# FedeMont/collision_handling_in_instantNGP

Measured on AMD Instinct MI355X. Metric: Mpixels/sec fwd+bwd at L=16,F=2,T=2^19, higher is better.
Workload: dtype f32

## Files before the change

collision_handling_in_instantngp_amd/_lib.py:

```python
import ctypes
import os

import torch

_HERE = os.path.dirname(os.path.abspath(__file__))
LIB_PATH = os.environ.get("GNGF_LIB_PATH") or os.path.join(_HERE, "libgngf_hip.so")

_c = ctypes
_P = _c.c_void_p
_I = _c.c_int
_L = _c.c_int64
_F = _c.c_float
_D = _c.c_double

SIGNATURES = {
    "gngf_abi_version": [],
    "gngf_hash_indices": [_P, _P, _P, _L, _I, _L, _P],
    "gngf_mrhe_fwd": [_P, _I, _P, _P, _P, _L, _I, _I, _L, _I, _I, _P],
    "gngf_mrhe_bwd": [_P, _I, _P, _P, _P, _P, _P, _L, _I, _I, _L, _I, _I, _P],
    "gngf_bilinear_fwd": [_P, _P, _P, _P, _L, _I, _I, _P],
    "gngf_bilinear_bwd": [_P, _P, _P, _P, _L, _I, _I, _P],
    "gngf_encode_fwd": [_P, _P, _I, _P, _P, _P, _P, _L, _I, _I, _L, _I, _I, _I, _L, _I, _I, _P, _P],
    "gngf_encode_bwd": [_P, _P, _I, _P, _P, _P, _P, _P, _P, _L, _I, _I, _L, _I, _I, _I, _L, _I, _I, _P],
    "gngf_encode_bwd_bucketed_plan": [_L, _I, _L, _I, _I, _P],
    "gngf_encode_bwd_bucketed": [_P, _P, _P, _P, _L, _I, _I, _L, _I, _I, _I, _I, _P, _P, _P, _P, _P],
    "gngf_clear_hashed_rows": [_P, _P, _I, _I, _L, _L, _P],
    "gngf_bin_pixels": [_P, _L, _I, _I, _I, _P, _P, _P, _P, _P, _P, _P],
    "gngf_encode_tiled_prepare": [_P, _L, _I, _I, _I, _P, _P, _P, _P, _P, _P, _P, _I, _P, _P, _P, _P, _P, _P, _I, _I, _I, _L, _I, _I, _I, _L,
                                  _P, _L, _P, _P, _P],
    "gngf_vertex_grid_fwd": [_P, _I, _P, _P, _P, _P, _P, _I, _I, _L, _I, _I, _I, _L, _P],
    "gngf_vertex_grid_bwd": [_P, _I, _P, _P, _P, _P, _P, _P, _P, _I, _I, _L, _I, _I, _I, _L, _P],
    "gngf_encode_tiled_fwd": [_P, _P, _P, _I, _P, _P, _P, _P, _I, _I, _I, _I, _I, _P],
    "gngf_bin_pixels2": [_P, _P, _L, _P],
    "gngf_encode_tiled_fwd_fused": [_P, _P, _P, _I, _P, _P, _P, _I, _P, _P, _P, _I, _I, _I, _L, _I, _I, _I, _L, _I, _I, _P, _P],
    "gngf_set_tiled_interleaved": [_I],
    "gngf_tiled_interleaved_applies": [_P, _I, _I, _I, _I, _I],
    "gngf_debug_il_stamps": [_P],
    "gngf_encode_tiled_bwd": [_P, _P, _P, _I, _P, _P, _P, _P, _P, _P, _I, _I, _P, _P, _I, _I, _I, _I, _I, _I,
                              _P, _P, _P, _P, _P, _P, _P, _L, _I, _I, _P, _P, _P, _P, _P, _P, _L, _P, _L, _P, _I, _P, _P],
    "gngf_vertex_grid_bwd_sorted": [_P, _I, _P, _P, _P, _P, _P, _P, _L, _P, _P, _I, _I, _L, _I, _I, _L, _P],
    "gngf_decoder_fwd": [_P, _P, _P, _P, _P, _P, _P, _P, _P, _L, _I, _I, _I, _P],
    "gngf_decoder_bwd": [_P, _P, _P, _P, _P, _P, _P, _P, _P, _P, _P, _P, _P, _P, _P, _P, _P, _P, _P, _P, _P, _L, _L, _I, _I, _I, _P],
    "gngf_decoder_reduce": [_P, _P, _P, _P, _P, _P, _P, _P, _P, _P, _L, _I, _I, _P],
    "gngf_decoder_train": [_P] * 20 + [_L, _L, _I, _I, _I, _P],
    "gngf_decoder_bwd_last_span_ns": [_P],
    "gngf_decoder_hidden_floats": [_L],
    "gngf_decoder_bwd_slabs": [_L],
    "gngf_decoder_slab_floats": [_I, _I],
    "gngf_set_gemm_split_bf16": [_I],
    "gngf_set_decoder_bwd_hybrid": [_I],
    "gngf_linear_fwd": [_P, _P, _P, _P, _L, _I, _I, _I, _P],
    "gngf_linear_bwd_input": [_P, _P, _P, _P, _L, _I, _I, _I, _P],
    "gngf_linear_bwd_weight": [_P, _P, _P, _P, _P, _L, _I, _I, _I, _P],
    "gngf_gemm_acc": [_P, _P, _P, _L, _L, _L, _I, _I, _P],
    "gngf_softmax_topk": [_P, _P, _P, _P, _L, _L, _I, _P],
    "gngf_softmax_bwd_lowrank": [_P, _P, _P, _P, _P, _P, _I, _P, _P, _P, _L, _L, _I, _P],
    "gngf_hpd_bwd_dot": [_P, _P, _P, _P, _P, _P, _I, _P, _L, _L, _I, _P],
    "gngf_hpd_bwd_fused_applies": [_L, _L, _I, _I, _I],
    "gngf_hpd_bwd_prepare": [_P, _P, _L, _P, _P, _P, _P, _L, _P, _P, _I, _I, _I, _P],
    "gngf_hpd_bwd_fused": [_P] * 8 + [_L, _P, _P, _P, _P, _P, _P, _P, _L, _L, _I, _I, _I, _P],
    "gngf_logits_topk_pbar": [_P, _P, _P, _P, _P, _I, _P, _L, _L, _I, _P],
    "gngf_linear_fwd_rowstats": [_P, _P, _P, _P, _P, _L, _I, _I, _P],
    "gngf_rowstats_topk": [_P, _P, _P, _P, _P, _L, _L, _I, _P],
    "gngf_pbar_accumulate": [_P, _P, _P, _I, _P, _L, _L, _P],
    "gngf_topk": [_P, _P, _P, _L, _L, _I, _P],
    "gngf_softmax_bwd": [_P, _P, _P, _P, _P, _P, _I, _P, _L, _L, _I, _P],
    "gngf_vertex_coords": [_P, _L, _L, _I, _P],
    "gngf_blend_fwd": [_P, _P, _L, _I, _I, _P],
    "gngf_blend_bwd": [_P, _P, _P, _L, _I, _I, _P],
    "gngf_vertex_multiplicity": [_P, _P, _P, _L, _I, _I, _L, _P],
    "gngf_multiplicity_weights": [_P, _P, _L, _I, _F, _P],
    "gngf_expand_vertex_table": [_P, _P, _P, _P, _P, _P, _P, _L, _I, _I, _I, _L, _P],
    "gngf_mse_workspace_floats": [],
# ... 101 lines not shown
```

collision_handling_in_instantngp_amd/csrc/encode_tiled.hip:

```cpp
#include "gngf_common.h"

namespace gngf {

#ifndef GNGF_TBF
#define GNGF_TBF 512
#endif
#ifndef GNGF_TBB
#define GNGF_TBB 1024
#endif
constexpr int kTBF = GNGF_TBF;
constexpr int kTB = GNGF_TBB;
#ifndef GNGF_BIN_THREADS
#define GNGF_BIN_THREADS 1024
#endif
constexpr int kBinThreads = GNGF_BIN_THREADS;
constexpr int kBinU = 8;

__device__ __forceinline__ int g_max0(int v) { return v < 0 ? 0 : v; }

__device__ __forceinline__ int tile_of(float x, float y, int tile_shift) {
  const int TS = 1 << tile_shift;
  int tx = (int)(x * (float)TS), ty = (int)(y * (float)TS);
  tx = tx < 0 ? 0 : (tx >= TS ? TS - 1 : tx);
  ty = ty < 0 ? 0 : (ty >= TS ? TS - 1 : ty);
// ... 1501 lines not shown
      y = dppf<0x114, 0xF>(x); asm volatile("" : "+v"(y)); x += p4 ? y : 0.f;
      y = dppf<0x118, 0xF>(x); asm volatile("" : "+v"(y)); x += p8 ? y : 0.f;
      y = dppf<0x142, 0xA>(x); asm volatile("" : "+v"(y)); x += pA ? y : 0.f;
      y = dppf<0x143, 0xC>(x); asm volatile("" : "+v"(y)); x += pB ? y : 0.f;
      v[f] = x;
    }
    float (*tail)[F] = s_tail[l & 1];
    if (lane == 63) {
#pragma unroll
      for (int f = 0; f < F; ++f) tail[wave][f] = v[f];
    }
    __syncthreads();
    float carry[F];
#pragma unroll
    for (int f = 0; f < F; ++f) carry[f] = 0.f;
    for (int q = wave - 1; q >= 0; --q) {
      if (s_last[q] != first_key) break;
#pragma unroll
      for (int f = 0; f < F; ++f) carry[f] += tail[q][f];
      if (s_nruns[q] != 1) break;
    }
    if (emit) {
      float* d = dtables + ((int64_t)l * T + slot) * F;
#pragma unroll
      for (int f = 0; f < F; ++f) {
        const float tot = v[f] + (in_first_run ? carry[f] : 0.f);
        if (tot != 0.f) atomicAdd(d + f, tot);
      }
    }
  }
  if (live && dvert_w) dvert_w[e] = dw_acc;
}

}

using namespace gngf;

#define DISPATCH_TT(dt, ...)                                                          \
  if ((dt) == GNGF_FEAT_F32) { using TT = float; __VA_ARGS__; }                       \
  else if ((dt) == GNGF_FEAT_F16) { using TT = __half; __VA_ARGS__; }                 \
  else return (int)hipErrorInvalidValue;

#define DISPATCH_F(F, ...)                          \
  switch (F) {                                      \
    case 1: { constexpr int kF = 1; __VA_ARGS__; } break; \
    case 2: { constexpr int kF = 2; __VA_ARGS__; } break; \
    case 4: { constexpr int kF = 4; __VA_ARGS__; } break; \
    case 8: { constexpr int kF = 8; __VA_ARGS__; } break; \
    default: return (int)hipErrorInvalidValue;      \
  }

static bool bin_job_dev(const gngf_bin_job* j, bool reserving, BinJobDev* d) {
  if (!j || j->P < 0 || j->P >= (1ll << 31) || j->tile_shift < 0 || j->tile_shift > 6 || j->NB <= 0 || j->NB > kBinMaxBlocks || j->chunk <= 0)
    return false;
  if (!(j->xy && j->blockhist && j->tile_off && j->tile_item_base && j->items && j->n_items && j->sorted)) return false;
  if (reserving && !(j->P > 0 && j->persistent_ws)) return false;
  d->xy = reinterpret_cast<const float2*>(j->xy); d->P = j->P;
  d->per_block = ceil_div(ceil_div(j->P, j->NB), kBinThreads) * kBinThreads;
  d->NB = j->NB; d->tile_shift = j->tile_shift; d->chunk = j->chunk;
  d->blockhist = j->blockhist; d->pws = j->persistent_ws; d->tile_off = j->tile_off; d->tile_item_base = j->tile_item_base;
  d->items = reinterpret_cast<int4*>(j->items); d->n_items = j->n_items; d->sorted = reinterpret_cast<float4*>(j->sorted);
  return true;
}
static BinJobDev bin_job_none() {
  BinJobDev d = {nullptr, 0, 0, 0, 0, 0, nullptr, nullptr, nullptr, nullptr, nullptr, nullptr, nullptr};
  return d;
// ... 365 lines not shown
    if (max_items > 0 && !hdt_g) {
      if (hash_dtables)
        gather_partials_kernel<kF, true><<<dim3((unsigned)ceil_div(vtot_h, 256)), dim3(256), 0, as_stream(stream)>>>(
            partials, tile_item_base, tile_level_off, n_ls, dG, Ls, tile_shift, lds_bytes / 4, hash_dtables, hash_T, hpow2);
      else
        gather_partials_kernel<kF><<<dim3((unsigned)ceil_div(vtot_h, 256)), dim3(256), 0,
                                     as_stream(stream)>>>(partials, tile_item_base, tile_level_off, n_ls, dG, Ls, tile_shift,
                                                          lds_bytes / 4);
    }
  });
  GNGF_RETURN_LAUNCH();
}

extern "C" int gngf_vertex_grid_bwd_sorted(const void* tables, int feat_dtype, const int32_t* vert_idx, const float* vert_w,
                                           const int32_t* order, const int32_t* n_ls, const float* dG, const void* dG64,
                                           int64_t vtot, float* dtables, float* dvert_w, int Ls, int F, int64_t T, int K,
                                           int vstride, int64_t NV, void* stream) {
  GNGF_CHECK_ARG(Ls > 0 && Ls <= GNGF_MAX_LEVELS && T > 0 && K > 0 && K <= GNGF_MAX_TOPK && vstride > 0 && NV > 0);
  GNGF_CHECK_ARG(tables && vert_idx && vert_w && order && n_ls && (dG || (dG64 && vtot > 0)) && dtables && NV * K < (1ll << 31));
  const int64_t NE = NV * K;
  if (dG64) {
    DISPATCH_TT(feat_dtype, DISPATCH_F(F, (vertex_bwd_sorted_kernel<kF, TT, true><<<dim3((unsigned)ceil_div(NE, kVB)), dim3(kVB), 0,
                                                                                  as_stream(stream)>>>(
                                static_cast<const TT*>(tables), vert_idx, vert_w, order, n_ls, nullptr, dtables, dvert_w, Ls, T, K,
                                vstride, NE, static_cast<const unsigned long long*>(dG64), vtot))));
    GNGF_RETURN_LAUNCH();
  }
  DISPATCH_TT(feat_dtype, DISPATCH_F(F, (vertex_bwd_sorted_kernel<kF, TT, false><<<dim3((unsigned)ceil_div(NE, kVB)), dim3(kVB), 0,
                                                                                 as_stream(stream)>>>(
                              static_cast<const TT*>(tables), vert_idx, vert_w, order, n_ls, dG, dtables, dvert_w, Ls, T, K,
                              vstride, NE, nullptr, 0))));
  GNGF_RETURN_LAUNCH();
}
```

collision_handling_in_instantngp_amd/models.py:

```python
from typing import Tuple

import numpy as np
import torch
import torch.nn as nn

from . import ops
from .params import *

device = torch.device("cuda") if torch.cuda.is_available() else torch.device("cpu")

DENSE_OUTPUT_LIMIT_BYTES = 4 << 30
HPD_CHUNK_BYTES = 8 << 30


def level_resolutions(n_min: int, n_max: int, num_levels: int) -> np.ndarray:
    b = np.exp((np.log(n_max) - np.log(n_min)) / (num_levels - 1))
    return np.array([np.floor(n_min * b ** l) for l in range(num_levels)]).astype(np.int32)


class DifferentiableTopk(torch.autograd.Function):

    @staticmethod
    def forward(ctx, input: torch.Tensor, k: int, dim: int):
        if dim not in (-1, input.dim() - 1):
# ... 216 lines not shown
                self._fused_mse_target, self._fused_mse_gloss = prev
        return scope()

    def _vertex_extent(self, x):
        if self.coord_bounds is not None:
            mx, my = self.coord_bounds
        else:
            if x.shape[0] > 0:
                b = torch.cat([x.amax(0), -x.amin(0)])
            else:
                b = torch.zeros((4,), dtype=x.dtype, device=x.device)
            if self.dp.max_ is not None:
                self.dp.max_(b)
            mx, my, nx, ny = b.tolist()
            if nx > 0 or ny > 0:
                raise ValueError("GNGF indexing builds its per-vertex table over [0, max] x [0, max]: negative coordinates "
                                 f"(min {-nx:g}, {-ny:g}) are outside it")
        gx_hi = int(np.floor(np.float32(mx) * np.float32(self._n_max))) + 1
        gy_hi = int(np.floor(np.float32(my) * np.float32(self._n_max))) + 1
        return gx_hi + 1, (gx_hi + 1) * (gy_hi + 1)

    def hpd_is_frozen(self):
        return all(not p.requires_grad for p in self.HPD.parameters())

    @torch.no_grad()
    def _frozen_vertex_table(self, blend_code):
        params = self.HPD.flat_params()
        key = (tuple((p.data_ptr(), p._version) for p in params), blend_code, self._topk_k)
        if self._frozen_table is None or self._frozen_table[0] != key:
            vstride = self._n_max + 2
            NV = vstride * vstride
            tv, ti, _, _ = ops.HpdVertexFunction.apply(NV, vstride, self._topk_k, None, False, HPD_CHUNK_BYTES, None, *params)
            w = ops.BlendFunction.apply(tv, blend_code)
            self._frozen_table = (key, tv, ti, w, vstride, NV, ops.slot_order(ti, self._n_ls_host, vstride))
            if self._row_map is not None:
                self._mark_reachable_rows(ti, vstride, NV)
        return self._frozen_table[1:]

    @torch.no_grad()
    def _mark_reachable_rows(self, vert_idx, vstride, NV):
        import ctypes
        from ._lib import call, ptr, stream_ptr
        L = self._num_levels
        dev = self._row_map.device
        host = (ctypes.c_int32 * L)(*self._n_ls_host)
        K = 1 if vert_idx is None else int(vert_idx.shape[1])
        call("gngf_mark_reachable_rows", ptr(self._n_ls_flat(dev), torch.int32), host, L, ptr(vert_idx, torch.int32), K,
             self._hash_table_size, int(vstride), int(NV), ptr(self._row_map), stream_ptr())

    def reachable_rows(self):
        if should_batchnorm_data:
            return None
        frozen = None
        if not self._hash_mode:
            cached = self._should_keep_topk_only or (self.dense_probs is False and not self.compute_pbar)
            if not (self.hpd_is_frozen() and cached):
                return None
            frozen = ops.BLEND_CODES[should_softmax_topk_features]
        dev = self.encoding._hash_tables[0].weight.device
        if not dev.type == "cuda":
            return None
        fresh = self._row_map is None or self._row_map.device != dev
        if fresh:
            from ._lib import query
            L, T = self._num_levels, self._hash_table_size
            assert query("gngf_slot_bitmap_words", L, 1, T) == L * ((T + 31) // 32)
            self._row_map = torch.zeros((L, (T + 31) // 32), dtype=torch.int32, device=dev)
# ... 210 lines not shown
```

collision_handling_in_instantngp_amd/ops.py:

```python
import ctypes as _ct
import dataclasses as _dc
import math as _math
import os
import sys as _sys
import types as _types

import torch

from . import _lib
from ._lib import call, ptr, query, stream_ptr

BLEND_CODES = {True: 0, None: 1, False: 2}
MODE_HASH, MODE_VERTEX_TABLE = 0, 1

_f32, _i32, _i64 = torch.float32, torch.int32, torch.int64


@_dc.dataclass(frozen=True)
class Tuning:
    fp16_table_grad_fp32: bool = False
    persistent_table_grad: bool = True
    persistent_min_bytes: int = 1 << 28
    bucketed_direct_bwd: bool = True
    bucketed_min_pixels: int = 1 << 16
# ... 986 lines not shown
def _vertex_fwd(plan, tables, vert_idx, vert_w, n_ls, vstride, G):
    L, T, F = tables.shape
    mode = MODE_HASH if vert_idx is None else MODE_VERTEX_TABLE
    call("gngf_vertex_grid_fwd", *_tab(tables), ptr(vert_idx), ptr(vert_w), ptr(n_ls), plan.n_ls_c, ptr(G), plan.Ls, F, T,
         0 if vert_idx is None else vert_idx.shape[1], mode, vstride, 0 if vert_idx is None else vert_idx.shape[0], stream_ptr())


_FIRST_LEVEL_KEYS = {}


def _first_level_keys(n_ls_host, vstride, NV, K, device):
    key = (n_ls_host, vstride, NV, K, str(device))
    hit = _FIRST_LEVEL_KEYS.get(key)
    if hit is None:
        if len(_FIRST_LEVEL_KEYS) > 16:
            _FIRST_LEVEL_KEYS.clear()
        vid = torch.arange(NV, device=device, dtype=_i64)
        m = torch.maximum(vid % vstride, vid // vstride)
        lmin = torch.zeros_like(m)
        for n in n_ls_host:
            lmin += (m > n + 1).to(_i64)
        hit = _FIRST_LEVEL_KEYS[key] = (lmin << 32).repeat_interleave(K)
    return hit


def slot_order(vert_idx, n_ls_host=None, vstride=None):
    NV, K = vert_idx.shape
    flat = vert_idx.reshape(-1).to(_i64)
    if n_ls_host is not None and vstride:
        flat = _first_level_keys(tuple(int(n) for n in n_ls_host), int(vstride), int(NV), int(K), vert_idx.device) | flat
    return torch.sort(flat, stable=True)[1].to(_i32)


_TILE_LEVEL_OFF = {}


def tile_level_offsets(plan, device):
    key = (tuple(plan.n_ls_host[:plan.Ls]), plan.tile_shift, plan.lds_bytes, plan.F, str(device))
    hit = _TILE_LEVEL_OFF.get(key)
    if hit is None:
        import numpy as np
        s, ts = plan.tile_shift, 1 << plan.tile_shift
        t = np.arange(ts * ts, dtype=np.int64)
        tx, ty = t & (ts - 1), t >> s
        lo = np.zeros(ts * ts, dtype=np.int64)
        out = np.full((ts * ts, plan.Ls), -1, dtype=np.int32)
        cap = plan.lds_bytes // 4
        for l, n in enumerate(plan.n_ls_host[:plan.Ls]):
            cx, cy = (tx * n) >> s, (ty * n) >> s
            hx = np.minimum((((tx + 1) * n) >> s) + 1, n + 1)
            hy = np.minimum((((ty + 1) * n) >> s) + 1, n + 1)
            sz = (hx - cx + 1) * (hy - cy + 1) * plan.F
            fits = lo + sz <= cap
            out[fits, l] = lo[fits]
            lo = np.where(fits, lo + sz, lo)
        hit = torch.from_numpy(out).to(device)
        _TILE_LEVEL_OFF[key] = hit
    return hit


STEP_CHAIN_SIGNATURE = "r5: [bin_count_ride+bin_scatter2 | riders of the previous step] > tiled_fwd_il<SRC tables>(+count riders) > decoder_train > tiled_bwd_il(+scatter tasks, reduce, mse)<hash: HDT, table rows added by the store pass> [> vertex_bwd_sorted<FROM64> (vertex-table source)]"


PIXEL_BWD_TRACE = None


def _pixel_bwd(plan, ws, n_ls, genc, dG, L, F, absmax=None, link=None, hash_fuse=None, dG64=None, next_bin=None):
    if PIXEL_BWD_TRACE is not None:
        PIXEL_BWD_TRACE.append({"P": plan.P, "Ls": plan.Ls, "bound": absmax is not None, "dG64": dG64 is not None and absmax is not None,
                                "hash_fuse": hash_fuse is not None, "fp32_grid": dG is not None,
                                "direct_hash": hash_fuse is not None and dG is None and dG64 is None,
                                "interleaved": plan.interleaved(backward=True)})
    partials = torch.empty((plan.max_items * (plan.lds_bytes // 4),), dtype=_f32, device=genc.device)
    am, am_count, am_stride = absmax if absmax is not None else (None, 0, 0)
    ride = link.take_reduce(genc.device) if link is not None else None
    if ride is None:
        ride_args = [ptr(None)] * 7 + [0, 0, 0]
    else:
        ride_args = [ptr(ride["slabs"])] + [_ct.c_void_p(a) for a in ride["gptrs"]] + [ride["P"], ride["in_dim"], ride["out_dim"]]
    ride_args += list(link.promise_ptrs()) if link is not None else [ptr(None), ptr(None)]
    lv = link.take_loss_value(genc.device) if link is not None else None
    if lv is None:
        ride_args += [ptr(None)] * 4 + [0]
    else:
        ride_args += [ptr(lv["pred"]), ptr(lv["label"]), ptr(lv["loss"]), ptr(lv["ws"]), lv["pred"].numel()]
    ride_args += [ptr(hash_fuse[0], _f32, "dtables"), int(hash_fuse[1])] if hash_fuse is not None else [ptr(None), 0]
    ride_args += [ptr(dG64, _i64, "dG64"), max(1, int(plan.P - 1).bit_length())] if dG64 is not None else [ptr(None), 0]
    ride_args += [_ct.byref(next_bin) if next_bin is not None else None]
    call("gngf_encode_tiled_bwd", ptr(ws.sorted), ptr(ws.items), ptr(ws.n_items), plan.max_items, ptr(ws.tile_item_base),
         ptr(tile_level_offsets(plan, genc.device)), ptr(n_ls), plan.n_ls_c, ptr(genc, _f32, "grad"), ptr(am),
         int(am_count), int(am_stride), ptr(dG), ptr(partials), L, plan.Ls, F, plan.tile_shift, plan.lds_bytes, plan.chunk,
         *ride_args, stream_ptr())


def run_deferred_vertex_stage(dp, exchanged=False):
    if dp is None or dp.deferred is None:
        return False
    plan, tables, vert_idx, vert_w, n_ls, vstride, dG, dtables, order, gout = dp.deferred
    if dp.exchange is not None and not exchanged:
        dp.exchange(dG)
    _vertex_bwd(plan, tables, vert_idx, vert_w, n_ls, vstride, dG, dtables, None, order)
    if gout is not None and gout is not dtables:
        gout[:plan.Ls].copy_(dtables[:plan.Ls])
    return True


def _vertex_bwd(plan, tables, vert_idx, vert_w, n_ls, vstride, dG, dtables, dvw, order=None, dG64=None):
    L, T, F = tables.shape
    if vert_idx is not None and order is not None:
        call("gngf_vertex_grid_bwd_sorted", *_tab(tables), ptr(vert_idx), ptr(vert_w), ptr(order, _i32, "order"), ptr(n_ls), ptr(dG),
             ptr(dG64, _i64, "dG64"), plan.vtot, ptr(dtables), ptr(dvw), plan.Ls, F, T, vert_idx.shape[1], vstride, vert_idx.shape[0],
             stream_ptr())
        return
    if dG64 is not None:
        raise ValueError("the fixed-point vertex grid is read by the slot-ordered vertex backward only")
    mode = MODE_HASH if vert_idx is None else MODE_VERTEX_TABLE
    call("gngf_vertex_grid_bwd", *_tab(tables), ptr(vert_idx), ptr(vert_w), ptr(n_ls), plan.n_ls_c, ptr(dG), ptr(dtables), ptr(dvw),
         plan.Ls, F, T, 0 if vert_idx is None else vert_idx.shape[1], mode, vstride,
         0 if vert_idx is None else vert_idx.shape[0], stream_ptr())


_SIDE_STREAMS = {}


def _side_stream(device):
    if not TUNING.use_side_stream:
        return torch.cuda.current_stream(device)
    key = (device.type, device.index, torch.cuda.current_stream(device).stream_id)
    if key not in _SIDE_STREAMS:
        _SIDE_STREAMS[key] = torch.cuda.Stream(device=device)
    return _SIDE_STREAMS[key]


@_dc.dataclass(frozen=True)
class StepConfig:
    source: str
    staged: int
    direct: int
    binning: str
    vertex_fwd: str
    pixel: str
    grad_sink: str
    table_grad: str
    clear: str
    direct_bwd: str
    exchange: bool

    def signature(self):
        return (f"{self.source} L{self.staged}+{self.direct} bin={self.binning} vfwd={self.vertex_fwd} px={self.pixel} sink={self.grad_sink} "
                f"dE={self.table_grad}/{self.clear} direct={self.direct_bwd}" + (" xchg" if self.exchange else ""))

    def chain(self):
        lv = ("tiled" if self.staged else "") + ("+" if self.staged and self.direct else "") + ("direct" if self.direct else "")
        return (f"{self.source} {lv} bin={self.binning} vfwd={self.vertex_fwd} px={self.pixel} sink={self.grad_sink} "
                f"dE={self.table_grad}/{self.clear} direct={self.direct_bwd}" + (" xchg" if self.exchange else ""))

    @staticmethod
    def choose(plan, L, T, F, P, mode, fp32_tables, needs_grad, link_defer_zero, link_zero_hidden, exchange, persist_ok, persist_alloc_ok,
               have_reserve_ws):
        t = TUNING
        src = "hash" if mode == MODE_HASH else "vertex_table"
        tiled = plan.Ls > 0 and P > 0
        nd = L - plan.Ls
        if not tiled:
            return StepConfig(src, 0, L, "none", "none", "none", "none", "alloc" if needs_grad else "none", "none",
                              "bucketed_or_atomics" if (needs_grad and nd > 0) else "none", False)
        il_f, il_b = plan.interleaved(backward=False), plan.interleaved(backward=True)
        fused = bool(t.fused_vertex_fwd and have_reserve_ws and fp32_tables and F == 2 and il_f)
        if needs_grad and (L * T * F) % 4 != 0:
            fused = False
        if not needs_grad:
            vf0 = "fused" if (fused or (t.fused_vertex_fwd and mode == MODE_HASH and not il_f)) else "riders"
            return StepConfig(src, plan.Ls, nd, "pipeline" if fused else "prepare", vf0,
                              "interleaved" if il_f else "generic", "none", "none", "none", "none", bool(exchange))
        use64 = F == 2 and plan.Ls <= 16 and il_b
        sink = "table_rows" if (mode == MODE_HASH and not exchange) else ("dG64" if use64 else "fp32_grid")
        if fused:
            return StepConfig(src, plan.Ls, nd, "pipeline", "fused", "interleaved", sink, "block", "decoder" if link_defer_zero else "riders",
                              "bucketed_or_atomics" if nd > 0 else "none", bool(exchange))
        fresh = nd > 0 and mode == MODE_HASH and bucketed_plan(P, F, T, nd, True) is not None
        hidden = link_defer_zero and link_zero_hidden and L * T * F * 4 <= t.persistent_min_bytes
        persist = bool(t.persistent_table_grad and not hidden and mode == MODE_HASH and persist_ok and not exchange and (fresh or nd == 0)
                       and persist_alloc_ok)
        vf = "fused" if (t.fused_vertex_fwd and mode == MODE_HASH and not il_f) else "riders"
        return StepConfig(src, plan.Ls, nd, "prepare", vf, "interleaved" if il_b else "generic", sink,
                          "persist" if persist else "alloc", "rows" if persist else ("decoder" if link_defer_zero else "riders"),
                          "bucketed_write" if fresh else ("bucketed_or_atomics" if nd > 0 else "none"), bool(exchange))


@_dc.dataclass
class _BackwardBuffers:
    dgrid: object = None
    dtables: object = None
    zbuf: object = None
    persist_cleared: object = None
    next_bin: object = None


class EncodeFunction(torch.autograd.Function):

    @staticmethod
    def forward(ctx, xy, n_ls, plan, tables, vert_idx, vert_w, vstride, order=None, dp=None, link=None, sink=None):
        ctx.dp, ctx.link, ctx.sink = dp, link, sink
        xy, tables = _c(xy), _c(tables)
        L, T, F = tables.shape
        P = xy.shape[0]
        mode = MODE_HASH if vert_idx is None else MODE_VERTEX_TABLE
        K = 0 if vert_idx is None else vert_idx.shape[1]
        NV = 0 if vert_idx is None else vert_idx.shape[0]
        enc = torch.empty((P, L * F), dtype=_f32, device=tables.device)
        ws = None
        if vert_idx is not None and order is None and plan.Ls > 0 and P > 0 and ctx.needs_input_grad[3]:
            order = slot_order(vert_idx, plan.n_ls_host[:plan.Ls], vstride)
        buf = None
        clear_now = None
        dev = tables.device
        tiled = plan.Ls > 0 and P > 0
        pws = _bin_workspace(dev, plan.ntiles, dp, kind="reserve") if (tiled and TUNING.fused_vertex_fwd) else None
        sc = ctx.step_config = StepConfig.choose(
            plan, L, T, F, P, mode, tables.dtype == _f32, bool(ctx.needs_input_grad[3]),
            bool(link is not None and link.defer_zero), bool(link is not None and link.zero_hidden),
            bool(dp is not None and dp.exchange is not None), bool(dp is not None and dp.persist_ok and getattr(dp, "level_params", None)),
            bool(dp is not None and (getattr(dp, "persist_grad", None) is not None or not torch.cuda.is_current_stream_capturing())),
            bool(pws is not None and pws.numel() >= 2 * plan.ntiles + 3))
        if dp is not None:
            dp.step_config = sc
        _trace("step_config", signature=sc.signature())
        if SEEN_STEP_CONFIGS is not None:
            SEEN_STEP_CONFIGS.add(sc.chain())
        if tiled:
            fused = sc.vertex_fwd == "fused" and sc.binning == "pipeline"
            use64 = sc.grad_sink == "dG64"
            if ctx.needs_input_grad[3]:
                ng = 0 if sc.grad_sink == "table_rows" else ((plan.vtot * F + 2) * 2 if use64 else plan.vtot * F)
                nt = tables.numel()
                if fused:
                    big = torch.empty((nt + ((ng + 3) & ~3),), dtype=_f32, device=dev)
                    dgrid = None if ng == 0 else (big[nt:nt + ng].view(_i64) if use64 else big[nt:nt + ng].view(plan.vtot, F))
                    buf = _BackwardBuffers(dgrid, big[:nt].view(tables.shape), zbuf=big)
                else:
                    dgrid = None if ng == 0 else (torch.empty((plan.vtot * F + 2,), dtype=_i64, device=dev) if use64
                                                  else torch.empty((plan.vtot, F), dtype=_f32, device=dev))
                    if sc.table_grad == "persist":
                        clear_now = _persistent_peek(dp, tables)
                        buf = _BackwardBuffers(dgrid, persist_cleared=dp.persist_gen if clear_now is not None else None)
                    else:
                        dt_ = torch.empty(tables.shape, dtype=_f32, device=dev)
                        buf = _BackwardBuffers(dgrid, dt_, zbuf=dt_[:plan.Ls] if sc.direct_bwd == "bucketed_write" else dt_)
                tile_level_offsets(plan, dev)
            zbuf = None if buf is None else buf.zbuf
            defer = zbuf is not None and link is not None and link.defer_zero and zbuf.numel() % 4 == 0
            if defer:
                link.zero_request = zbuf
            if fused:
                pipe = dp.pipeline if (dp is not None and TUNING.bin_pipeline) else None
                if pipe is not None and pipe.pending is not None:
                    pipe.pending = None
# ... 68 lines not shown
            dtables = _persistent_grad(dp, tables, plan, n_ls, buf.persist_cleared)
        _trace("table_grad", source=("persist" if (dtables is not None and dp is not None and dtables is getattr(dp, "persist_grad", None))
                                     else ("forward_alloc" if dtables is not None else "zeroed_alloc")))
        fresh_direct = dtables is not None and sc.direct_bwd == "bucketed_write"
        if dtables is None:
            dtables = _grad_buffer(tables)
        dvw = torch.zeros_like(vert_w) if (vert_w is not None and ctx.needs_input_grad[5]) else None
        if plan.Ls > 0 and P > 0:
            fuse = (dtables, T) if (vert_idx is None and exchange is None) else None
            direct_hash = grad_sink == "table_rows" and fuse is not None
            dG64 = dgrid if grad_sink == "dG64" else None
            direct64 = dG64 is not None and vert_idx is not None and order is not None and exchange is None and dvw is None
            if direct64 or direct_hash:
                dG = None
            elif dG64 is None and dgrid is not None:
                dG = dgrid
            else:
                dG = (torch.empty if dG64 is not None else torch.zeros)((plan.vtot, F), dtype=_f32, device=tables.device)
            next_bin = None if buf is None else buf.next_bin
            job_next = None
            if next_bin is not None and plan.interleaved(backward=True):
                job_next = next_bin[1]
            _pixel_bwd(plan, ws, n_ls, genc, dG, L, F, absmax, link, fuse, dG64, job_next)
            if job_next is not None:
                ws_next, _job, nx, pipe = next_bin
                pipe.ready = (BinPipeline._key(nx, plan), ws_next)
                if pipe.pending is ws_next:
                    pipe.pending = None
            if fuse is None and exchange is not None and dp.defer_vertex and dvw is None:
                if plan.Ls < L:
                    _direct_bwd(xy, tables, vert_idx, vert_w, n_ls, genc, dtables, dvw, P, L, F, T, K, mode, vstride, NV, plan.Ls, L,
                                fresh=fresh_direct, order=(ws.sorted if ws is not None else None))
                gout = _grad_out(dtables, tables, sink)
                dp.deferred = (plan, tables, vert_idx, vert_w, n_ls, vstride, dG, dtables, order, gout)
                dp.tables_reduced = plan.Ls
                return (None, None, None, gout, None, dvw, *NONE)
            if exchange is not None:
                exchange(dG)
                dp.tables_reduced = plan.Ls
            if fuse is not None:
                dvw_t = None
            elif order is not None and dvw is not None and plan.Ls < L:
                dvw_t = torch.empty_like(dvw)
                _vertex_bwd(plan, tables, vert_idx, vert_w, n_ls, vstride, dG, dtables, dvw_t, order)
            else:
                dvw_t = None
                _vertex_bwd(plan, tables, vert_idx, vert_w, n_ls, vstride, dG, dtables, dvw, order, dG64 if direct64 else None)
        else:
            dvw_t = None
        if plan.Ls < L:
            _direct_bwd(xy, tables, vert_idx, vert_w, n_ls, genc, dtables, dvw, P, L, F, T, K, mode, vstride, NV, plan.Ls, L,
                        fresh=fresh_direct, order=(ws.sorted if ws is not None else None))
        if dvw_t is not None:
            dvw = dvw + dvw_t
        return (None, None, None, _grad_out(dtables, tables, sink), None, dvw, *NONE)


def encode_apply(xy, n_ls, n_ls_host, tables, vert_idx, vert_w, vstride, path=None, order=None, dp=None, link=None, sink=None):
    plan = EncodePlan(xy.shape[0], n_ls_host, tables.shape[2], path)
    return EncodeFunction.apply(xy, n_ls, plan, tables, vert_idx, vert_w, vstride, order, dp, link, sink)


_MSE_WORKSPACE = {}


class MseFunction(torch.autograd.Function):

    @staticmethod
    def forward(ctx, pred, label):
        pred, label = _c(pred), _c(label)
        if pred.shape != label.shape:
            raise ValueError(f"pred {tuple(pred.shape)} and label {tuple(label.shape)} differ")
        if pred.numel() == 0:
            raise ValueError("MSE of an empty batch")
        dev = pred.device
        ws = _MSE_WORKSPACE.get(dev)
        if ws is None:
            ws = _MSE_WORKSPACE[dev] = torch.zeros(query("gngf_mse_workspace_floats"), dtype=_f32, device=dev)
        loss = torch.empty((), dtype=_f32, device=dev)
        call("gngf_mse_fwd", ptr(pred, _f32, "pred"), ptr(label, _f32, "label"), ptr(loss), ptr(ws), pred.numel(), stream_ptr())
# ... 369 lines not shown
```

include/gngf.h:

```cpp
#ifndef GNGF_H_
#define GNGF_H_

#include <stdint.h>

#ifdef __cplusplus
extern "C" {
#endif

#define GNGF_ABI_VERSION 14
#define GNGF_MAX_LEVELS 32
#define GNGF_MAX_TOPK 32

enum { GNGF_BLEND_SOFTMAX = 0 , GNGF_BLEND_RAW = 1 , GNGF_BLEND_NORM = 2  };

enum { GNGF_FEAT_F32 = 0, GNGF_FEAT_F16 = 1 };

enum { GNGF_MODE_HASH = 0 , GNGF_MODE_VERTEX_TABLE = 1  };

int gngf_abi_version(void);

int gngf_hash_indices(const float* xy, const int32_t* n_ls, int64_t* idx, int64_t P, int L, int64_t T, void* stream);

int gngf_mrhe_fwd(const void* tables, int feat_dtype, const int64_t* idx, const float* probs, float* out,
                  int64_t P, int L, int F, int64_t T, int K, int blend, void* stream);
// ... 41 lines not shown
  int32_t* blockhist;
  int32_t* persistent_ws;
  int32_t* tile_off;
  int32_t* tile_item_base;
  int32_t* items;
  int32_t* n_items;
  float* sorted;
} gngf_bin_job;
int gngf_bin_pixels2(const gngf_bin_job* job, float* zero_fill, int64_t zero_floats, void* stream);
int gngf_encode_tiled_fwd_fused(const float* sorted, const int32_t* items, const int32_t* n_items, int max_items,
                                const int32_t* n_ls, const int32_t* n_ls_host, const void* tables, int feat_dtype,
                                const int32_t* vert_idx, const float* vert_w, float* enc, int L, int Ls, int F, int64_t T, int K,
                                int mode, int vstride, int64_t NV, int tile_shift, int lds_bytes, const gngf_bin_job* next_count,
                                void* stream);
int gngf_encode_tiled_fwd(const float* sorted, const int32_t* items, const int32_t* n_items, int max_items,
                          const int32_t* n_ls, const int32_t* n_ls_host, const float* G, float* enc, int L, int Ls, int F,
                          int tile_shift, int lds_bytes, void* stream);
int gngf_set_tiled_interleaved(int on);
int gngf_tiled_interleaved_applies(const int32_t* n_ls_host, int Ls, int F, int tile_shift, int lds_bytes, int backward);
int gngf_debug_il_stamps(unsigned long long* host8);
int gngf_encode_tiled_bwd(const float* sorted, const int32_t* items, const int32_t* n_items, int max_items,
                          const int32_t* tile_item_base, const int32_t* tile_level_off, const int32_t* n_ls,
                          const int32_t* n_ls_host, const float* genc, const float* genc_absmax, int absmax_count,
                          int absmax_stride, float* dG, float* partials, int L, int Ls, int F, int tile_shift, int lds_bytes,
                          int chunk, const float* ride_slabs, float* ride_dW0, float* ride_db0, float* ride_dW1, float* ride_db1,
                          float* ride_dW2, float* ride_db2, int64_t ride_P, int ride_in_dim, int ride_out_dim,
                          const float* gloss_promised, const float* gloss_arrived,
                          const float* mse_pred, const float* mse_label, float* mse_loss, float* mse_workspace, int64_t mse_n,
                          float* hash_dtables, int64_t hash_T, void* dG64, int log2_pixels, const gngf_bin_job* next_bin,
                          void* stream);
int gngf_vertex_grid_bwd_sorted(const void* tables, int feat_dtype, const int32_t* vert_idx, const float* vert_w, const int32_t* order,
                                const int32_t* n_ls, const float* dG, const void* dG64, int64_t vtot, float* dtables, float* dvert_w,
                                int Ls, int F, int64_t T, int K, int vstride, int64_t NV, void* stream);

int gngf_set_gemm_split_bf16(int mode);
int gngf_set_decoder_bwd_hybrid(int on);
int gngf_decoder_train(const float* enc, const float* target, const float* gloss, const float* W0, const float* b0,
                       const float* W1, const float* b1, const float* W2, const float* b2, float* rgb, float* denc,
                       float* dW0, float* db0, float* dW1, float* db1, float* dW2, float* db2, float* slabs,
                       float* denc_absmax, float* zero_fill, int64_t zero_floats, int64_t P, int in_dim, int out_dim, int leaky,
                       void* stream);
int gngf_linear_fwd(const float* X, const float* W, const float* b, float* Y, int64_t M, int N, int K, int act, void* stream);
int gngf_linear_bwd_input(const float* dY, const float* Y, const float* W, float* dX, int64_t M, int N, int K, int act,
                          void* stream);
int gngf_linear_bwd_weight(const float* dY, const float* Y, const float* X, float* dW, float* db, int64_t M, int N, int K,
                           int act, void* stream);
int gngf_gemm_acc(const float* A, const float* B, float* C, int64_t M, int64_t N, int64_t Kc, int ta, int tb, void* stream);

int gngf_decoder_fwd(const float* enc, const float* W0, const float* b0, const float* W1, const float* b1, const float* W2,
                     const float* b2, float* rgb, float* hidden, int64_t P, int in_dim, int out_dim, int leaky, void* stream);
int64_t gngf_decoder_hidden_floats(int64_t P);
int gngf_decoder_bwd(const float* enc, const float* rgb, const float* drgb, const float* target, const float* gloss,
                     const float* W0, const float* b0, const float* W1,
                     const float* b1, const float* W2, float* denc, float* dW0, float* db0, float* dW1, float* db1, float* dW2,
                     float* db2, float* slabs, float* denc_absmax, const float* hidden, float* zero_fill, int64_t zero_floats,
                     int64_t P, int in_dim, int out_dim, int leaky, void* stream);
int gngf_decoder_reduce(const float* slabs, float* dW0, float* db0, float* dW1, float* db1, float* dW2, float* db2,
                        float* denc_absmax, const float* gloss_promised, const float* gloss_arrived, int64_t P, int in_dim,
                        int out_dim, void* stream);
int gngf_decoder_bwd_slabs(int64_t P);
int gngf_decoder_bwd_last_span_ns(double* ns);
int gngf_decoder_slab_floats(int in_dim, int out_dim);

int gngf_softmax_topk(float* logits_probs, float* topk_val, int32_t* topk_idx, float* rowstat, int64_t U, int64_t T, int K,
                      void* stream);
int gngf_logits_topk_pbar(const float* logits, float* topk_val, int32_t* topk_idx, float* rowstat, const float* mw, int L,
// ... 84 lines not shown
```

Measured before the change: 2549.

## Add flat destination-sorted item list kernel for frozen vertex-table backward

Builds, once per frozen vertex table, a static list of (grid vertex, weight, destination row) items sorted by destination, and adds a kernel that streams it with vector loads. The kernel does a segmented scan within each block and issues one atomic per destination run, replacing the sorted-order vertex backward kernel. This is meant to cut the indirection and atomic traffic of the per-step scatter into the hash tables. In exchange it adds host-side list construction, extra memory for the list, and a fallback path when the list exceeds its size cap or is built during stream capture.

```diff
diff --git a/collision_handling_in_instantngp_amd/_lib.py b/collision_handling_in_instantngp_amd/_lib.py
--- a/collision_handling_in_instantngp_amd/_lib.py
+++ b/collision_handling_in_instantngp_amd/_lib.py
@@ -39,6 +39,7 @@
     "gngf_encode_tiled_bwd": [_P, _P, _P, _I, _P, _P, _P, _P, _P, _P, _I, _I, _P, _P, _I, _I, _I, _I, _I, _I,
                               _P, _P, _P, _P, _P, _P, _P, _L, _I, _I, _P, _P, _P, _P, _P, _P, _L, _P, _L, _P, _I, _P, _P],
     "gngf_vertex_grid_bwd_sorted": [_P, _I, _P, _P, _P, _P, _P, _P, _L, _P, _P, _I, _I, _L, _I, _I, _L, _P],
+    "gngf_vertex_grid_bwd_flat": [_P, _P, _P, _L, _P, _P, _L, _P, _L, _I, _P],
     "gngf_decoder_fwd": [_P, _P, _P, _P, _P, _P, _P, _P, _P, _L, _I, _I, _I, _P],
     "gngf_decoder_bwd": [_P, _P, _P, _P, _P, _P, _P, _P, _P, _P, _P, _P, _P, _P, _P, _P, _P, _P, _P, _P, _P, _L, _L, _I, _I, _I, _P],
     "gngf_decoder_reduce": [_P, _P, _P, _P, _P, _P, _P, _P, _P, _P, _L, _I, _I, _P],
diff --git a/collision_handling_in_instantngp_amd/csrc/encode_tiled.hip b/collision_handling_in_instantngp_amd/csrc/encode_tiled.hip
--- a/collision_handling_in_instantngp_amd/csrc/encode_tiled.hip
+++ b/collision_handling_in_instantngp_amd/csrc/encode_tiled.hip
@@ -1557,6 +1557,150 @@
   if (live && dvert_w) dvert_w[e] = dw_acc;
 }
 
+constexpr int kFlatTB = 256;
+constexpr int kFlatIPT = 4;
+static_assert(kFlatIPT % 4 == 0 && kFlatTB % 64 == 0, "whole 16-byte loads, whole waves");
+template <int F, bool FROM64>
+__global__ void __launch_bounds__(kFlatTB)
+vertex_bwd_flat_kernel(const int32_t* __restrict__ item_gi, const float* __restrict__ item_w, const int32_t* __restrict__ item_dest,
+                       int64_t N, const float* __restrict__ dG, const unsigned long long* __restrict__ dG64, int64_t vtot,
+                       float* __restrict__ dtables, int64_t rows) {
+  constexpr int NW = kFlatTB / 64;
+  __shared__ int s_firstd[kFlatTB], s_lastd[kFlatTB];
+  __shared__ float s_y[kFlatTB][F];
+  __shared__ float s_wtot[NW][F];
+  __shared__ int s_wflag[NW];
+  const int tid = threadIdx.x, lane = tid & 63, wave = tid >> 6;
+  const int64_t i0 = ((int64_t)blockIdx.x * kFlatTB + tid) * kFlatIPT;
+  int gi[kFlatIPT], d[kFlatIPT];
+  float w[kFlatIPT];
+  if (i0 + kFlatIPT <= N) {
+#pragma unroll
+    for (int c = 0; c < kFlatIPT; c += 4) {
+      const int4 g4 = *reinterpret_cast<const int4*>(item_gi + i0 + c);
+      const float4 w4 = *reinterpret_cast<const float4*>(item_w + i0 + c);
+      const int4 d4 = *reinterpret_cast<const int4*>(item_dest + i0 + c);
+      gi[c] = g4.x; gi[c + 1] = g4.y; gi[c + 2] = g4.z; gi[c + 3] = g4.w;
+      w[c] = w4.x; w[c + 1] = w4.y; w[c + 2] = w4.z; w[c + 3] = w4.w;
+      d[c] = d4.x; d[c + 1] = d4.y; d[c + 2] = d4.z; d[c + 3] = d4.w;
+    }
+  } else {
+#pragma unroll
+    for (int i = 0; i < kFlatIPT; ++i) {
+      const bool on = i0 + i < N;
+      gi[i] = on ? item_gi[i0 + i] : 0;
+      w[i] = on ? item_w[i0 + i] : 0.f;
+      d[i] = on ? item_dest[i0 + i] : -1;
+    }
+  }
+  float v[kFlatIPT][F];
+  if constexpr (FROM64) {
+    unsigned long long q[kFlatIPT][F];
+#pragma unroll
+    for (int i = 0; i < kFlatIPT; ++i) {
+      const int64_t g = gi[i] < 0 ? 0 : (gi[i] < vtot ? gi[i] : vtot - 1);
+#pragma unroll
+      for (int f = 0; f < F; ++f) q[i][f] = dG64[g * F + f];
+    }
+    const double inv64 = ldexp(1.0, -(int)(long long)dG64[vtot * F]);
+    const bool poisoned = dG64[vtot * F + 1] != 0ull;
+#pragma unroll
+    for (int i = 0; i < kFlatIPT; ++i)
+#pragma unroll
+      for (int f = 0; f < F; ++f)
+        v[i][f] = (poisoned ? __int_as_float(0x7fc00000) : (float)((double)(long long)q[i][f] * inv64)) * w[i];
+  } else {
+    float q[kFlatIPT][F];
+#pragma unroll
+    for (int i = 0; i < kFlatIPT; ++i) {
+      const int64_t g = gi[i] < 0 ? 0 : (gi[i] < vtot ? gi[i] : vtot - 1);
+#pragma unroll
+      for (int f = 0; f < F; ++f) q[i][f] = dG[g * F + f];
+    }
+#pragma unroll
+    for (int i = 0; i < kFlatIPT; ++i)
+#pragma unroll
+      for (int f = 0; f < F; ++f) v[i][f] = q[i][f] * w[i];
+  }
+  auto emit = [&](int dest, const float* s) {
+    if ((uint64_t)(int64_t)dest < (uint64_t)rows) {
+      float* p = dtables + (int64_t)dest * F;
+#pragma unroll
+      for (int f = 0; f < F; ++f)
+        if (s[f] != 0.f) atomicAdd(p + f, s[f]);
+    }
+  };
+  float acc[F], head[F];
+  int nb = 0;
+#pragma unroll
+  for (int f = 0; f < F; ++f) { acc[f] = v[0][f]; head[f] = 0.f; }
+#pragma unroll
+  for (int i = 1; i < kFlatIPT; ++i) {
+    if (d[i] != d[i - 1]) {
+      if (nb == 0) {
+#pragma unroll
+        for (int f = 0; f < F; ++f) head[f] = acc[f];
+      } else {
+        emit(d[i - 1], acc);
+      }
+      ++nb;
+#pragma unroll
+      for (int f = 0; f < F; ++f) acc[f] = v[i][f];
+    } else {
+#pragma unroll
+      for (int f = 0; f < F; ++f) acc[f] += v[i][f];
+    }
+  }
+  s_firstd[tid] = d[0];
+  s_lastd[tid] = d[kFlatIPT - 1];
+  __syncthreads();
+  const int prev_d = tid > 0 ? s_lastd[tid - 1] : -2;
+  const int next_d = tid + 1 < kFlatTB ? s_firstd[tid + 1] : -2;
+  const int starts = (nb > 0 || prev_d != d[0]) ? 1 : 0;
+  float y[F];
+  int flag = starts;
+#pragma unroll
+  for (int f = 0; f < F; ++f) y[f] = acc[f];
+#pragma unroll
+  for (int o = 1; o < 64; o <<= 1) {
+    const int fu = __shfl_up(flag, o, 64);
+    float yu[F];
+#pragma unroll
+    for (int f = 0; f < F; ++f) yu[f] = __shfl_up(y[f], o, 64);
+    if (lane >= o) {
+      if (!flag) {
+#pragma unroll
+        for (int f = 0; f < F; ++f) y[f] += yu[f];
+      }
+      flag |= fu;
+    }
+  }
+  if (lane == 63) {
+#pragma unroll
+    for (int f = 0; f < F; ++f) s_wtot[wave][f] = y[f];
+    s_wflag[wave] = flag;
+  }
+  __syncthreads();
+  if (!flag) {
+    for (int q = wave - 1; q >= 0; --q) {
+#pragma unroll
+      for (int f = 0; f < F; ++f) y[f] += s_wtot[q][f];
+      if (s_wflag[q]) break;
+    }
+  }
+#pragma unroll
+  for (int f = 0; f < F; ++f) s_y[tid][f] = y[f];
+  __syncthreads();
+  if (nb > 0) {
+    if (tid > 0 && prev_d == d[0]) {
+#pragma unroll
+      for (int f = 0; f < F; ++f) head[f] += s_y[tid - 1][f];
+    }
+    emit(d[0], head);
+  }
+  if (next_d != d[kFlatIPT - 1]) emit(d[kFlatIPT - 1], y);
+}
+
 }
 
 using namespace gngf;
@@ -1988,3 +2132,20 @@
                               vstride, NE, nullptr, 0))));
   GNGF_RETURN_LAUNCH();
 }
+
+extern "C" int gngf_vertex_grid_bwd_flat(const int32_t* item_gi, const float* item_w, const int32_t* item_dest, int64_t N,
+                                         const float* dG, const void* dG64, int64_t vtot, float* dtables, int64_t rows, int F,
+                                         void* stream) {
+  GNGF_CHECK_ARG(item_gi && item_w && item_dest && N > 0 && N < (1ll << 31) && (dG || dG64) && vtot > 0 && dtables);
+  GNGF_CHECK_ARG(rows > 0 && rows < (1ll << 31));
+  GNGF_CHECK_ARG(((reinterpret_cast<uintptr_t>(item_gi) | reinterpret_cast<uintptr_t>(item_w) | reinterpret_cast<uintptr_t>(item_dest)) & 15) == 0);
+  const dim3 grid((unsigned)ceil_div(N, (int64_t)kFlatTB * kFlatIPT)), block(kFlatTB);
+  if (dG64) {
+    DISPATCH_F(F, (vertex_bwd_flat_kernel<kF, true><<<grid, block, 0, as_stream(stream)>>>(
+                      item_gi, item_w, item_dest, N, nullptr, static_cast<const unsigned long long*>(dG64), vtot, dtables, rows)));
+    GNGF_RETURN_LAUNCH();
+  }
+  DISPATCH_F(F, (vertex_bwd_flat_kernel<kF, false><<<grid, block, 0, as_stream(stream)>>>(item_gi, item_w, item_dest, N, dG, nullptr,
+                                                                                         vtot, dtables, rows)));
+  GNGF_RETURN_LAUNCH();
+}
diff --git a/collision_handling_in_instantngp_amd/models.py b/collision_handling_in_instantngp_amd/models.py
--- a/collision_handling_in_instantngp_amd/models.py
+++ b/collision_handling_in_instantngp_amd/models.py
@@ -272,7 +272,9 @@
             NV = vstride * vstride
             tv, ti, _, _ = ops.HpdVertexFunction.apply(NV, vstride, self._topk_k, None, False, HPD_CHUNK_BYTES, None, *params)
             w = ops.BlendFunction.apply(tv, blend_code)
-            self._frozen_table = (key, tv, ti, w, vstride, NV, ops.slot_order(ti, self._n_ls_host, vstride))
+            order = ops.attach_flat_lists(ops.slot_order(ti, self._n_ls_host, vstride), ti, w, self._n_ls_host, vstride,
+                                          self._hash_table_size)
+            self._frozen_table = (key, tv, ti, w, vstride, NV, order)
             if self._row_map is not None:
                 self._mark_reachable_rows(ti, vstride, NV)
         return self._frozen_table[1:]
diff --git a/collision_handling_in_instantngp_amd/ops.py b/collision_handling_in_instantngp_amd/ops.py
--- a/collision_handling_in_instantngp_amd/ops.py
+++ b/collision_handling_in_instantngp_amd/ops.py
@@ -1042,6 +1042,77 @@
     return torch.sort(flat, stable=True)[1].to(_i32)
 
 
+VERTEX_BWD_FLAT = 1
+VERTEX_BWD_FLAT_MAX_ITEMS = 1 << 22
+
+
+@_dc.dataclass(frozen=True)
+class VertexFlatList:
+    gi: object
+    w: object
+    dest: object
+    n: int
+    Ls: int
+    T: int
+    vtot: int
+
+
+def vertex_flat_list(vert_idx, vert_w, n_ls_host, vstride, T):
+    NV, K = vert_idx.shape
+    n_ls_host = [int(n) for n in n_ls_host]
+    Ls, vstride, T = len(n_ls_host), int(vstride), int(T)
+    vtot = sum((n + 2) * (n + 2) for n in n_ls_host)
+    if Ls == 0 or vtot * K > VERTEX_BWD_FLAT_MAX_ITEMS:
+        return None
+    if Ls * T >= 2 ** 31:
+        raise ValueError(f"vertex_flat_list: {Ls} levels of {T} rows do not fit a 32-bit row number")
+    dev = vert_idx.device
+    vids, lvls = [], []
+    for l, n in enumerate(n_ls_host):
+        gw = n + 2
+        if gw > vstride or (gw - 1) * vstride + gw > NV:
+            raise ValueError(f"vertex_flat_list: level {l}'s {gw} x {gw} vertex grid does not fit a table of {NV} vertices, stride {vstride}")
+        a = torch.arange(gw, device=dev, dtype=_i64)
+        vids.append((a[:, None] * vstride + a[None, :]).reshape(-1))
+        lvls.append(torch.full((gw * gw,), l, device=dev, dtype=_i64))
+    vid, lvl = torch.cat(vids), torch.cat(lvls)
+    slot = vert_idx[vid].to(_i64)
+    lo, hi = int(slot.min()), int(slot.max())
+    if lo < 0 or hi >= T:
+        raise ValueError(f"vertex_flat_list: slots span [{lo}, {hi}], outside the table's [0, {T})")
+    dest, perm = torch.sort((lvl[:, None] * T + slot).reshape(-1), stable=True)
+    gi = torch.arange(vtot, device=dev, dtype=_i64).repeat_interleave(K)[perm]
+    w = vert_w.detach()[vid].reshape(-1)[perm].to(_f32)
+    n = vtot * K
+    assert gi.numel() == w.numel() == dest.numel() == n
+    if int(gi.min()) < 0 or int(gi.max()) >= vtot or int(dest[0]) < 0 or int(dest[-1]) >= Ls * T:
+        raise ValueError("vertex_flat_list: an index left its range")
+    return VertexFlatList(gi.to(_i32).contiguous(), w.contiguous(), dest.to(_i32).contiguous(), n, Ls, T, vtot)
+
+
+class VertexFlatLists:
+
+    def __init__(self, vert_idx, vert_w, n_ls_host, vstride, T):
+        self.vert_idx, self.vert_w = vert_idx, vert_w
+        self.n_ls_host, self.vstride, self.T = [int(n) for n in n_ls_host], int(vstride), int(T)
+        self._lists = {}
+
+    def get(self, Ls, vert_idx, vert_w, T):
+        if vert_idx is not self.vert_idx or vert_w is not self.vert_w or int(T) != self.T or Ls > len(self.n_ls_host):
+            return None
+        if Ls not in self._lists:
+            if vert_idx.is_cuda and torch.cuda.is_current_stream_capturing():
+                return None
+            self._lists[Ls] = vertex_flat_list(vert_idx, vert_w, self.n_ls_host[:Ls], self.vstride, self.T)
+        return self._lists[Ls]
+
+
+def attach_flat_lists(order, vert_idx, vert_w, n_ls_host, vstride, T):
+    if order is not None:
+        order.flat_lists = VertexFlatLists(vert_idx, vert_w, n_ls_host, vstride, T)
+    return order
+
+
 _TILE_LEVEL_OFF = {}
 
 
@@ -1069,7 +1140,7 @@
     return hit
 
 
-STEP_CHAIN_SIGNATURE = "r5: [bin_count_ride+bin_scatter2 | riders of the previous step] > tiled_fwd_il<SRC tables>(+count riders) > decoder_train > tiled_bwd_il(+scatter tasks, reduce, mse)<hash: HDT, table rows added by the store pass> [> vertex_bwd_sorted<FROM64> (vertex-table source)]"
+STEP_CHAIN_SIGNATURE = "r6: [bin_count_ride+bin_scatter2 | riders of the previous step] > tiled_fwd_il<SRC tables>(+count riders) > decoder_train > tiled_bwd_il(+scatter tasks, reduce, mse)<hash: HDT, table rows added by the store pass> [> vertex_bwd_flat<FROM64> over the static item list of the frozen table (vertex-table source; vertex_bwd_sorted<FROM64> without a list)]"
 
 
 PIXEL_BWD_TRACE = None
@@ -1106,17 +1177,30 @@
 def run_deferred_vertex_stage(dp, exchanged=False):
     if dp is None or dp.deferred is None:
         return False
-    plan, tables, vert_idx, vert_w, n_ls, vstride, dG, dtables, order, gout = dp.deferred
+    plan, tables, vert_idx, vert_w, n_ls, vstride, dG, dtables, order, gout, flat = dp.deferred
     if dp.exchange is not None and not exchanged:
         dp.exchange(dG)
-    _vertex_bwd(plan, tables, vert_idx, vert_w, n_ls, vstride, dG, dtables, None, order)
+    _vertex_bwd(plan, tables, vert_idx, vert_w, n_ls, vstride, dG, dtables, None, order, **({"flat": flat} if flat is not None else {}))
     if gout is not None and gout is not dtables:
         gout[:plan.Ls].copy_(dtables[:plan.Ls])
     return True
 
 
-def _vertex_bwd(plan, tables, vert_idx, vert_w, n_ls, vstride, dG, dtables, dvw, order=None, dG64=None):
+def _flat_list_of(order, plan, vert_idx, vert_w, T):
+    lists = getattr(order, "flat_lists", None) if order is not None else None
+    if lists is None or not VERTEX_BWD_FLAT or vert_idx is None or plan.Ls <= 0:
+        return None
+    return lists.get(plan.Ls, vert_idx, vert_w, T)
+
+
+def _vertex_bwd(plan, tables, vert_idx, vert_w, n_ls, vstride, dG, dtables, dvw, order=None, dG64=None, flat=None):
     L, T, F = tables.shape
+    if flat is not None and dvw is None and VERTEX_BWD_FLAT and vert_idx is not None and order is not None:
+        if (flat.Ls, flat.T, flat.vtot) != (plan.Ls, T, plan.vtot):
+            raise ValueError(f"the item list is for {flat.Ls} levels of {flat.T} rows, {flat.vtot} vertices: not this plan's")
+        call("gngf_vertex_grid_bwd_flat", ptr(flat.gi, _i32, "item_gi"), ptr(flat.w, _f32, "item_w"), ptr(flat.dest, _i32, "item_dest"),
+             flat.n, ptr(dG), ptr(dG64, _i64, "dG64"), plan.vtot, ptr(dtables, _f32, "dtables"), plan.Ls * T, F, stream_ptr())
+        return
     if vert_idx is not None and order is not None:
         call("gngf_vertex_grid_bwd_sorted", *_tab(tables), ptr(vert_idx), ptr(vert_w), ptr(order, _i32, "order"), ptr(n_ls), ptr(dG),
              ptr(dG64, _i64, "dG64"), plan.vtot, ptr(dtables), ptr(dvw), plan.Ls, F, T, vert_idx.shape[1], vstride, vert_idx.shape[0],
@@ -1155,10 +1239,12 @@
     clear: str
     direct_bwd: str
     exchange: bool
+    vertex_bwd_flat: bool = False
 
     def signature(self):
         return (f"{self.source} L{self.staged}+{self.direct} bin={self.binning} vfwd={self.vertex_fwd} px={self.pixel} sink={self.grad_sink} "
-                f"dE={self.table_grad}/{self.clear} direct={self.direct_bwd}" + (" xchg" if self.exchange else ""))
+                f"dE={self.table_grad}/{self.clear} direct={self.direct_bwd}" + (" xchg" if self.exchange else "")
+                + (" vbwd=flat" if self.vertex_bwd_flat else ""))
 
     def chain(self):
         lv = ("tiled" if self.staged else "") + ("+" if self.staged and self.direct else "") + ("direct" if self.direct else "")
@@ -1167,7 +1253,7 @@
 
     @staticmethod
     def choose(plan, L, T, F, P, mode, fp32_tables, needs_grad, link_defer_zero, link_zero_hidden, exchange, persist_ok, persist_alloc_ok,
-               have_reserve_ws):
+               have_reserve_ws, flat_list=False):
         t = TUNING
         src = "hash" if mode == MODE_HASH else "vertex_table"
         tiled = plan.Ls > 0 and P > 0
@@ -1184,10 +1270,11 @@
             return StepConfig(src, plan.Ls, nd, "pipeline" if fused else "prepare", vf0,
                               "interleaved" if il_f else "generic", "none", "none", "none", "none", bool(exchange))
         use64 = F == 2 and plan.Ls <= 16 and il_b
+        vflat = bool(flat_list and mode != MODE_HASH)
         sink = "table_rows" if (mode == MODE_HASH and not exchange) else ("dG64" if use64 else "fp32_grid")
         if fused:
             return StepConfig(src, plan.Ls, nd, "pipeline", "fused", "interleaved", sink, "block", "decoder" if link_defer_zero else "riders",
-                              "bucketed_or_atomics" if nd > 0 else "none", bool(exchange))
+                              "bucketed_or_atomics" if nd > 0 else "none", bool(exchange), vflat)
         fresh = nd > 0 and mode == MODE_HASH and bucketed_plan(P, F, T, nd, True) is not None
         hidden = link_defer_zero and link_zero_hidden and L * T * F * 4 <= t.persistent_min_bytes
         persist = bool(t.persistent_table_grad and not hidden and mode == MODE_HASH and persist_ok and not exchange and (fresh or nd == 0)
@@ -1195,7 +1282,7 @@
         vf = "fused" if (t.fused_vertex_fwd and mode == MODE_HASH and not il_f) else "riders"
         return StepConfig(src, plan.Ls, nd, "prepare", vf, "interleaved" if il_b else "generic", sink,
                           "persist" if persist else "alloc", "rows" if persist else ("decoder" if link_defer_zero else "riders"),
-                          "bucketed_write" if fresh else ("bucketed_or_atomics" if nd > 0 else "none"), bool(exchange))
+                          "bucketed_write" if fresh else ("bucketed_or_atomics" if nd > 0 else "none"), bool(exchange), vflat)
 
 
 @_dc.dataclass
@@ -1220,6 +1307,8 @@
         NV = 0 if vert_idx is None else vert_idx.shape[0]
         enc = torch.empty((P, L * F), dtype=_f32, device=tables.device)
         ws = None
+        ctx.flat = (_flat_list_of(order, plan, vert_idx, vert_w, T)
+                    if (P > 0 and ctx.needs_input_grad[3] and not ctx.needs_input_grad[5]) else None)
         if vert_idx is not None and order is None and plan.Ls > 0 and P > 0 and ctx.needs_input_grad[3]:
             order = slot_order(vert_idx, plan.n_ls_host[:plan.Ls], vstride)
         buf = None
@@ -1232,7 +1321,7 @@
             bool(link is not None and link.defer_zero), bool(link is not None and link.zero_hidden),
             bool(dp is not None and dp.exchange is not None), bool(dp is not None and dp.persist_ok and getattr(dp, "level_params", None)),
             bool(dp is not None and (getattr(dp, "persist_grad", None) is not None or not torch.cuda.is_current_stream_capturing())),
-            bool(pws is not None and pws.numel() >= 2 * plan.ntiles + 3))
+            bool(pws is not None and pws.numel() >= 2 * plan.ntiles + 3), flat_list=ctx.flat is not None)
         if dp is not None:
             dp.step_config = sc
         _trace("step_config", signature=sc.signature())
@@ -1367,7 +1456,7 @@
                     _direct_bwd(xy, tables, vert_idx, vert_w, n_ls, genc, dtables, dvw, P, L, F, T, K, mode, vstride, NV, plan.Ls, L,
                                 fresh=fresh_direct, order=(ws.sorted if ws is not None else None))
                 gout = _grad_out(dtables, tables, sink)
-                dp.deferred = (plan, tables, vert_idx, vert_w, n_ls, vstride, dG, dtables, order, gout)
+                dp.deferred = (plan, tables, vert_idx, vert_w, n_ls, vstride, dG, dtables, order, gout, ctx.flat)
                 dp.tables_reduced = plan.Ls
                 return (None, None, None, gout, None, dvw, *NONE)
             if exchange is not None:
@@ -1380,7 +1469,8 @@
                 _vertex_bwd(plan, tables, vert_idx, vert_w, n_ls, vstride, dG, dtables, dvw_t, order)
             else:
                 dvw_t = None
-                _vertex_bwd(plan, tables, vert_idx, vert_w, n_ls, vstride, dG, dtables, dvw, order, dG64 if direct64 else None)
+                _vertex_bwd(plan, tables, vert_idx, vert_w, n_ls, vstride, dG, dtables, dvw, order, dG64 if direct64 else None,
+                            **({"flat": ctx.flat} if ctx.flat is not None else {}))
         else:
             dvw_t = None
         if plan.Ls < L:
diff --git a/include/gngf.h b/include/gngf.h
--- a/include/gngf.h
+++ b/include/gngf.h
@@ -97,6 +97,8 @@
 int gngf_vertex_grid_bwd_sorted(const void* tables, int feat_dtype, const int32_t* vert_idx, const float* vert_w, const int32_t* order,
                                 const int32_t* n_ls, const float* dG, const void* dG64, int64_t vtot, float* dtables, float* dvert_w,
                                 int Ls, int F, int64_t T, int K, int vstride, int64_t NV, void* stream);
+int gngf_vertex_grid_bwd_flat(const int32_t* item_gi, const float* item_w, const int32_t* item_dest, int64_t N, const float* dG,
+                              const void* dG64, int64_t vtot, float* dtables, int64_t rows, int F, void* stream);
 
 int gngf_set_gemm_split_bf16(int mode);
 int gngf_set_decoder_bwd_hybrid(int on);
```

After: 2594, median of 6. 1.8% higher.
